# nickgreenquist/cu2rec

Measured on AMD Instinct MI355X. Metric: ratings/sec (SGD updates/sec), higher is better.
Workload: dtype f32

## Files before the change

### cu2rec_amd/csrc/blocksolve.hpp

```cpp
#pragma once

#include <functional>
#include <vector>

#include <hip/hip_runtime.h>

#include <cstddef>
#include <cstdint>

#include "hip_check.hpp"
#include "kernels.hpp"

namespace cu2rec {

constexpr int kBsLinks = 64;
constexpr int kBsTableStride = 2 * kBsLinks + 1;
constexpr int kBsTableFloats = 4 * kBsTableStride;
constexpr int kBsFactorFloats = 3 * 32 * 32;
constexpr int kBsRecFloats = kBsFactorFloats + kBsLinks;
constexpr int kBsCrossFloats = kBsLinks * kBsLinks;
constexpr int kBsMaxSlots = 63;

struct BsBlockDesc {
    int pos0;
    int n_valid;
    int chain;
    int m;
};

struct BsChainDesc {
    int begin, len;
    int blk0;
    int item;
};

struct BsIteration {
    const uint32_t *keys;
    const uint64_t *vals;
    int n_active;
    int n_hot;
    uint32_t item_mask;
    const BsChainDesc *chains;
    const BsBlockDesc *blocks;
    const int *walk_begin;
    const int *item_of_rank;
    const float *tables;
    float log2a, log2c;
    float *Mbuf;
    float *ebuf;
    float *qstart;
    int max_blocks;
    int launch_blocks;
    int la_ranks;
    int la_cap;
    int la_grid;
    float *Nbuf;
    unsigned *status;
    unsigned long long *solve_started;
    const unsigned long long *side_seq;
    unsigned long long side_target;
    unsigned long long *gram_done;
    unsigned long long wait_ticks;
};

float blocksolve_min_rate(float rate);
int blocksolve_lookahead_blocks(int blocks);
int blocksolve_hot_items(const std::vector<double> &rate, int n_active, int rank_limit);

class BlockSolve {
public:
    BlockSolve(int n_hot, const std::vector<double> &rate, double hot_rate, int n_active, int item_bits, int max_batch,
               const int *item_of_rank);
    ~BlockSolve();
    BlockSolve(const BlockSolve &) = delete;
    BlockSolve &operator=(const BlockSolve &) = delete;
    void plan(int slot, const uint32_t *sk, int nb, size_t stride, hipStream_t sched);
    void begin(const SgdArgs &a, hipStream_t stream);
    using SideChains = std::function<void(hipStream_t side, hipEvent_t stop)>;
    void iteration(const SgdArgs &a, int slot, int b, const uint32_t *keys, const uint64_t *vals, bool last, hipStream_t stream,
                   const SideChains &side);
    void join(hipStream_t stream);
    void end(hipStream_t stream);

    const int n_hot;

private:
    int n_active, item_bits, max_batch;
    const int *item_of_rank;
    int max_blocks;
    int launch_blocks;
    int la_ranks = 0;
    int la_cap = 0;
    DeviceBuffer<int> chain_begin[2], walk_begin[2];
    DeviceBuffer<BsChainDesc> chains[2];
    DeviceBuffer<BsBlockDesc> blocks[2];
    DeviceBuffer<float> tables, Mbuf, ebuf, qstart, Nbuf;
    int qstart_ld = 0;
    SgdHyper tables_for{};
    bool tables_valid = false;
    DeviceBuffer<unsigned long long> solve_started, gram_done, side_seq;
    unsigned long long gram_done_target = 0, started_total = 0, side_seq_host = 0;
    hipStream_t upd = nullptr;
    hipEvent_t ev_call = nullptr, ev_upd = nullptr, ev_gram = nullptr;
    BsIteration it{};
    bool device_join = false;
    bool upd_pending = false;
    unsigned *host_status = nullptr;
};

}
```

### cu2rec_amd/csrc/blocksolve_device.hpp

```cpp
#pragma once

#include <hip/hip_runtime.h>

#include "blocksolve.hpp"
#include "sgd_device.hpp"

namespace cu2rec {
namespace bs_dev {

using namespace dev;

constexpr int kB = kBsLinks;
constexpr int kTabAdel = 0, kTabCdel = kBsTableStride, kTabApow = 2 * kBsTableStride, kTabCpow = 3 * kBsTableStride;
constexpr int kH = 32;
constexpr int kMS = 36;

typedef float f32x4 __attribute__((ext_vector_type(4)));
typedef float f32x2 __attribute__((ext_vector_type(2)));
__device__ __forceinline__ f32x4 lds4(const float4 *p) { return *reinterpret_cast<const f32x4 *>(p); }
__device__ __forceinline__ f32x2 lo2(f32x4 v) { return __builtin_shufflevector(v, v, 0, 1); }
__device__ __forceinline__ f32x2 hi2(f32x4 v) { return __builtin_shufflevector(v, v, 2, 3); }
__device__ __forceinline__ f32x2 fma2(f32x2 a, f32x2 b, f32x2 c) { return __builtin_elementwise_fma(a, b, c); }
__device__ __forceinline__ f32x2 dup2(float v) { return f32x2{v, v}; }
typedef unsigned int u32x2 __attribute__((ext_vector_type(2)));

__device__ __forceinline__ unsigned ld_agent(const unsigned *p) {
    return __hip_atomic_load(p, __ATOMIC_RELAXED, __HIP_MEMORY_SCOPE_AGENT);
}
__device__ __forceinline__ unsigned long long ld_agent(const unsigned long long *p) {
    return __hip_atomic_load(p, __ATOMIC_RELAXED, __HIP_MEMORY_SCOPE_AGENT);
}

__device__ __forceinline__ float row_pair_sum(float v) {
    const u32x2 r = __builtin_amdgcn_permlane16_swap(__float_as_uint(v), __float_as_uint(v), false, false);
    return __uint_as_float(r.x) + __uint_as_float(r.y);
}

__device__ __forceinline__ float half_sum(float v) {
    const u32x2 r = __builtin_amdgcn_permlane32_swap(__float_as_uint(v), __float_as_uint(v), false, false);
    return __uint_as_float(r.x) + __uint_as_float(r.y);
}

__device__ __forceinline__ float lane_value(float v, int lane) {
    return __int_as_float(__builtin_amdgcn_readlane(__float_as_int(v), lane));
}

__device__ __forceinline__ float4 zero4() { return make_float4(0.f, 0.f, 0.f, 0.f); }

__device__ __forceinline__ bool chain_is_lookahead(const BsIteration &it, int chain, const BsChainDesc &cd) {
    const int nblk = (cd.len + kB - 1) / kB;
    return chain < it.la_ranks && nblk >= 2 && cd.blk0 + nblk <= it.la_cap;
}

}
}
```

### cu2rec_amd/csrc/blocksolve_gram.hpp

```cpp
#pragma once

#include "blocksolve_device.hpp"
#include "mfma_f32.hpp"

namespace cu2rec {
namespace bs_dev {

constexpr int kGramTabFloats = 2 * kB;
__host__ __device__ inline size_t gram_tile_float4s(int nslots) { return static_cast<size_t>(kB) * (nslots | 1); }

__host__ __device__ inline int gram_tab_offset(int RS) { return max(4 * kB * RS, 5 * kH * kMS); }
__host__ __device__ inline size_t gram_lds_bytes(int nslots, bool with_cross_blocks) {
    const size_t own = static_cast<size_t>(gram_tab_offset(nslots | 1) + kGramTabFloats + kB) * sizeof(float);
    const size_t cross = with_cross_blocks ? 2 * gram_tile_float4s(nslots) * sizeof(float4) : 0;
    return own > cross ? own : cross;
}

__device__ __forceinline__ void gram_block(const SgdArgs &a, const BsIteration &it, int g, float4 *bs_smem) {
    const int wave = threadIdx.x >> 6, lane = threadIdx.x & 63;
    const BsBlockDesc bd = it.blocks[g];
    if (bd.n_valid == 0) return;
    const int nslots = a.nslots, RS = nslots | 1;
    float4 *tile = bs_smem;
    float *Ms = reinterpret_cast<float *>(bs_smem);
    float *Ns = Ms + 2 * kH * kMS;
    float *tab = Ms + gram_tab_offset(RS);
    float *basev = tab + kGramTabFloats;
    const bool mine = lane < bd.n_valid;
    const uint64_t val = it.vals[bd.pos0 + min(lane, bd.n_valid - 1)];
    const int x = static_cast<int>(val >> 32);
    if (wave == 3) {
        const float r0 = (__uint_as_float(static_cast<uint32_t>(val)) - a.global_bias) - a.user_bias[x];
        basev[lane] = mine ? r0 : 0.f;
        tab[lane] = it.tables[kTabApow + lane];
        tab[kB + lane] = it.tables[kTabCpow + lane];
    }
    const int rsub = lane >> 3, cs = lane & 7;
    const int nch = (nslots + 7) >> 3;
    for (int c0 = 0; c0 < nch; c0 += 4) {
        float4 v[2][4];
#pragma unroll
        for (int pp = 0; pp < 2; ++pp) {
            const int xr = __shfl(x, 16 * wave + 8 * pp + rsub);
            const float4 *src = reinterpret_cast<const float4 *>(a.P + static_cast<size_t>(xr) * a.ldp);
#pragma unroll
            for (int c = 0; c < 4; ++c) v[pp][c] = src[min(8 * (c0 + c) + cs, nslots - 1)];
        }
#pragma unroll
        for (int pp = 0; pp < 2; ++pp) {
            const int row = 16 * wave + 8 * pp + rsub;
#pragma unroll
            for (int c = 0; c < 4; ++c) {
                const int slot = 8 * (c0 + c) + cs;
                if (slot < nslots) tile[row * RS + slot] = row < bd.n_valid ? v[pp][c] : zero4();
            }
        }
    }
    __syncthreads();
    const int k = lane & 31, h = lane >> 5;
    f32x16 acc;
#pragma unroll
    for (int i = 0; i < 16; ++i) acc[i] = 0.f;
    if (wave < 3) {
        const int S0 = (nslots + 1) >> 1;
        const float4 *ra = tile + (wave == 1 ? kH + k : k) * RS, *rb = tile + (wave == 0 ? k : kH + k) * RS;
        for (int c = 0; c < S0; c += 2) {
            float4 va[2], vb[2];
#pragma unroll
            for (int i = 0; i < 2; ++i) {
                const int slot = h * S0 + c + i;
                const bool ok = c + i < S0 && slot < nslots;
                const float4 t0 = ra[min(slot, nslots - 1)], t1 = rb[min(slot, nslots - 1)];
                va[i] = ok ? t0 : zero4();
                vb[i] = ok ? t1 : zero4();
            }
#pragma unroll
            for (int i = 0; i < 2; ++i) {
                const float pa[4] = {va[i].x, va[i].y, va[i].z, va[i].w}, pb[4] = {vb[i].x, vb[i].y, vb[i].z, vb[i].w};
#pragma unroll
                for (int e = 0; e < 4; ++e) acc = __builtin_amdgcn_mfma_f32_32x32x2f32(pa[e], pb[e], acc, 0, 0, 0);
            }
        }
    }
    __syncthreads();
    if (wave < 3) {
        const float lr = a.h.lr;
        const int K = (wave == 0 ? 0 : kH) + k;
        const int J0 = (wave == 1 ? kH : 0) + 4 * h;
        const bool row_ok = K < bd.n_valid;
        float *dst = Ns + (wave * kH + k) * kMS + 4 * h;
#pragma unroll
        for (int m = 0; m < 4; ++m) {
            f32x4 out;
#pragma unroll
            for (int e = 0; e < 4; ++e) {
                const int d = K - 1 - (J0 + 8 * m + e);
                const float fd = static_cast<float>(d);
                const float v = lr * (__builtin_amdgcn_exp2f(fd * it.log2c) + __builtin_amdgcn_exp2f(fd * it.log2a) * acc[4 * m + e]);
                out[e] = d >= 0 && row_ok ? v : 0.f;
            }
            *reinterpret_cast<f32x4 *>(dst + 8 * m) = out;
        }
    }
    __syncthreads();
    if (wave == 0) {
    float m[kH];
    {
        const float *Nh = Ns + h * kH * kMS;
        float4 cur[8], nxt[8];
        m[0] = k == 0 ? 1.f : 0.f;
        cur[0] = *reinterpret_cast<const float4 *>(Nh + kMS);
#pragma unroll
        for (int kk = 1; kk < kH; ++kk) {
            if (kk + 1 < kH) {
#pragma unroll
                for (int i4 = 0; i4 < (kk + 4) / 4; ++i4) nxt[i4] = *reinterpret_cast<const float4 *>(Nh + (kk + 1) * kMS + 4 * i4);
            }
            __builtin_amdgcn_sched_barrier(0);
            float s[4] = {kk == k ? 1.f : 0.f, 0.f, 0.f, 0.f};
#pragma unroll
            for (int i4 = 0; i4 < (kk + 3) / 4; ++i4) {
                const float nv[4] = {cur[i4].x, cur[i4].y, cur[i4].z, cur[i4].w};
#pragma unroll
                for (int e = 0; e < 4; ++e)
                    if (4 * i4 + e < kk) s[e] = __builtin_fmaf(-nv[e], m[4 * i4 + e], s[e]);
            }
            m[kk] = (s[0] + s[1]) + (s[2] + s[3]);
            __builtin_amdgcn_sched_barrier(0);
            if (kk + 1 < kH) {
#pragma unroll
                for (int i4 = 0; i4 < (kk + 4) / 4; ++i4) cur[i4] = nxt[i4];
            }
        }
    }
#pragma unroll
    for (int kk = 0; kk < kH; ++kk) Ms[(h * kH + kk) * kMS + k] = m[kk];
    __builtin_amdgcn_wave_barrier();
    f32x16 tacc, macc;
#pragma unroll
    for (int i = 0; i < 16; ++i) tacc[i] = macc[i] = 0.f;
    {
        const float4 *arow = reinterpret_cast<const float4 *>(Ns + (2 * kH + k) * kMS + 16 * h);
#pragma unroll
        for (int t4 = 0; t4 < 4; ++t4) {
            const float4 a4 = arow[t4];
            const float av[4] = {a4.x, a4.y, a4.z, a4.w};
#pragma unroll
            for (int e = 0; e < 4; ++e)
                tacc = __builtin_amdgcn_mfma_f32_32x32x2f32(av[e], Ms[(16 * h + 4 * t4 + e) * kMS + k], tacc, 0, 0, 0);
        }
        const float *mrow = Ms + (kH + k) * kMS + 4 * h;
#pragma unroll
        for (int t4 = 0; t4 < 4; ++t4) {
            const float4 a4 = *reinterpret_cast<const float4 *>(mrow + 8 * t4);
            const float av[4] = {a4.x, a4.y, a4.z, a4.w};
#pragma unroll
            for (int e = 0; e < 4; ++e) macc = __builtin_amdgcn_mfma_f32_32x32x2f32(av[e], tacc[4 * t4 + e], macc, 0, 0, 0);
        }
    }
#pragma unroll
    for (int reg = 0; reg < 16; ++reg) Ns[acc_row(reg, h) * kMS + k] = -macc[reg];
    }
    __syncthreads();
    float *rec = it.Mbuf + static_cast<size_t>(g) * kBsRecFloats;
    {
        const int t = threadIdx.x, row = t >> 3, c4 = t & 7;
        const float *src[3] = {Ms, Ns, Ms + kH * kMS};
#pragma unroll
        for (int q = 0; q < 3; ++q) *reinterpret_cast<f32x4 *>(rec + q * kH * kH + 4 * t) = *reinterpret_cast<const f32x4 *>(src[q] + row * kMS + 4 * c4);
        if (t < kB / 4) *reinterpret_cast<f32x4 *>(rec + kBsFactorFloats + 4 * t) = *reinterpret_cast<const f32x4 *>(basev + 4 * t);
    }
}

__device__ __forceinline__ void gram_cross_block(const SgdArgs &a, const BsIteration &it, int g, float4 *smem) {
    const BsBlockDesc bd = it.blocks[g];
    if (bd.n_valid == 0 || bd.m == 0 || !chain_is_lookahead(it, bd.chain, it.chains[bd.chain])) return;
    const int wave = threadIdx.x >> 6, lane = threadIdx.x & 63, k = lane & 31, h = lane >> 5;
    const int rt = wave >> 1, ct = wave & 1;
    const int nslots = a.nslots, RS = nslots | 1, S0 = (nslots + 1) >> 1;
    float4 *tile_c = smem, *tile_p = smem + kB * RS;
    {
        const int xc = static_cast<int>(it.vals[bd.pos0 + min(lane, bd.n_valid - 1)] >> 32);
        const int xp = static_cast<int>(it.vals[bd.pos0 - kB + lane] >> 32);
        const int rsub = lane >> 3, cs = lane & 7;
        const int nch = (nslots + 7) >> 3;
        for (int c0 = 0; c0 < nch; c0 += 2) {
            float4 vc[2][2], vp[2][2];
#pragma unroll
            for (int pp = 0; pp < 2; ++pp) {
                const int src_lane = 16 * wave + 8 * pp + rsub;
                const float4 *sc = reinterpret_cast<const float4 *>(a.P + static_cast<size_t>(__shfl(xc, src_lane)) * a.ldp);
                const float4 *sp = reinterpret_cast<const float4 *>(a.P + static_cast<size_t>(__shfl(xp, src_lane)) * a.ldp);
#pragma unroll
                for (int c = 0; c < 2; ++c) {
                    vc[pp][c] = sc[min(8 * (c0 + c) + cs, nslots - 1)];
                    vp[pp][c] = sp[min(8 * (c0 + c) + cs, nslots - 1)];
                }
            }
#pragma unroll
            for (int pp = 0; pp < 2; ++pp) {
                const int row = 16 * wave + 8 * pp + rsub;
#pragma unroll
                for (int c = 0; c < 2; ++c) {
                    const int slot = 8 * (c0 + c) + cs;
                    if (slot < nslots) {
                        tile_c[row * RS + slot] = row < bd.n_valid ? vc[pp][c] : zero4();
                        tile_p[row * RS + slot] = vp[pp][c];
                    }
                }
            }
        }
    }
    __syncthreads();
    f32x16 acc;
#pragma unroll
    for (int i = 0; i < 16; ++i) acc[i] = 0.f;
    {
        const float4 *ra = tile_c + (kH * rt + k) * RS, *rb = tile_p + (kH * ct + k) * RS;
        for (int c = 0; c < S0; c += 2) {
            float4 va[2], vb[2];
#pragma unroll
            for (int i = 0; i < 2; ++i) {
                const int slot = h * S0 + c + i;
                const bool ok = c + i < S0 && slot < nslots;
                const float4 t0 = ra[min(slot, nslots - 1)], t1 = rb[min(slot, nslots - 1)];
                va[i] = ok ? t0 : zero4();
                vb[i] = ok ? t1 : zero4();
            }
#pragma unroll
            for (int i = 0; i < 2; ++i) {
                const float pa[4] = {va[i].x, va[i].y, va[i].z, va[i].w}, pb[4] = {vb[i].x, vb[i].y, vb[i].z, vb[i].w};
#pragma unroll
                for (int e = 0; e < 4; ++e) acc = __builtin_amdgcn_mfma_f32_32x32x2f32(pa[e], pb[e], acc, 0, 0, 0);
            }
        }
    }
    const float lr = a.h.lr;
    float *dst = it.Nbuf + static_cast<size_t>(g) * kBsCrossFloats;
    const int j = kH * ct + k;
#pragma unroll
    for (int reg = 0; reg < 16; ++reg) {
        const int i = kH * rt + acc_row(reg, h);
        const float fd = static_cast<float>(kB - 1 + i - j);
        const float v = lr * (__builtin_amdgcn_exp2f(fd * it.log2c) + __builtin_amdgcn_exp2f(fd * it.log2a) * acc[reg]);
        dst[i * kB + j] = i < bd.n_valid ? v : 0.f;
    }
    __syncthreads();
}

}
}
```

### cu2rec_amd/csrc/blocksolve_lookahead.hpp

```cpp
#pragma once

#include "blocksolve_device.hpp"

namespace cu2rec {
namespace bs_dev {

constexpr int kLaPRing = 3, kLaRRing = 2, kLaDepth = 2;
constexpr int kLaNS4 = 17;
constexpr int kLaRec4 = 3 * kH * kMS / 4 + kB * kLaNS4;
constexpr int kLaQ4 = 32;
constexpr int kLaMaxSlots = 29;
__host__ __device__ inline bool la_supported(int nslots) { return nslots >= 1 && nslots <= kLaMaxSlots; }
__host__ __device__ inline size_t la_lds_bytes(int nslots) {
    return (static_cast<size_t>(kLaPRing) * kB * (nslots | 1) + kLaRRing * kLaRec4 + 2 * kLaQ4 + 7 * kB / 4 + (kBsTableFloats + 3) / 4 + 4 + 64) * 16;
}

enum { kSyC0 = 0, kSyC1 = 1, kSyE = 2, kSyG = 3, kSyLdP = 4, kSyLdR = 8, kSyR = 12, kSyAbort = 13 };

template <class Reached>
__device__ __forceinline__ void la_wait_until(unsigned *sy, const BsIteration &it, Reached reached) {
    unsigned polls = 0;
    unsigned long long t0 = 0;
    while (!reached()) {
        __builtin_amdgcn_s_sleep(1);
        if ((++polls & 1023u) == 0) {
            if (t0 == 0) t0 = wall_clock64();
            if (__hip_atomic_load(sy + kSyAbort, __ATOMIC_RELAXED, __HIP_MEMORY_SCOPE_WORKGROUP) != 0u || wall_clock64() - t0 > it.wait_ticks) {
                __hip_atomic_store(sy + kSyAbort, 2u, __ATOMIC_RELAXED, __HIP_MEMORY_SCOPE_WORKGROUP);
                if ((threadIdx.x & 63) == 0) __hip_atomic_store(it.status, 2u, __ATOMIC_RELAXED, __HIP_MEMORY_SCOPE_AGENT);
                break;
            }
        }
    }
    asm volatile("" ::: "memory");
}
__device__ __forceinline__ void la_wait(unsigned *sy, int word, unsigned target, const BsIteration &it) {
    la_wait_until(sy, it, [=] __device__ { return __hip_atomic_load(sy + word, __ATOMIC_RELAXED, __HIP_MEMORY_SCOPE_WORKGROUP) >= target; });
}
__device__ __forceinline__ void la_wait4(unsigned *sy, int word, unsigned target, const BsIteration &it) {
    la_wait_until(sy, it, [=] __device__ {
        typedef unsigned u32x4 __attribute__((ext_vector_type(4)));
        const u32x4 v = __builtin_nontemporal_load((const __attribute__((address_space(3))) u32x4 *)(sy + word));
        asm volatile("" ::: "memory");
        return min(min(v.x, v.y), min(v.z, v.w)) >= target;
    });
}
__device__ __forceinline__ void la_wait2(unsigned *sy, int word, unsigned target, const BsIteration &it) {
    la_wait_until(sy, it, [=] __device__ {
        const u32x2 v = __builtin_nontemporal_load((const __attribute__((address_space(3))) u32x2 *)(sy + word));
        asm volatile("" ::: "memory");
        return min(v.x, v.y) >= target;
    });
}
__device__ __forceinline__ void la_post(unsigned *sy, int word, unsigned value) {
    asm volatile("" ::: "memory");
    if ((threadIdx.x & 63) == 0) __hip_atomic_store(sy + word, value, __ATOMIC_RELAXED, __HIP_MEMORY_SCOPE_WORKGROUP);
}

template <int NSM>
__device__ __forceinline__ void chain_lookahead(const SgdArgs &a, const BsIteration &it, float4 *smem, const BsChainDesc &cd) {
    const int tid = threadIdx.x, wave = tid >> 6, lane = tid & 63;
    const int nslots = a.nslots, RS = nslots | 1;
    const int begin = cd.begin, len = cd.len, nblk = (len + kB - 1) / kB, g0 = cd.blk0, y = cd.item;
    float4 *pring = smem;
    float4 *rring = pring + kLaPRing * kB * RS;
    float4 *qbuf = rring + kLaRRing * kLaRec4;
    float *wbuf = reinterpret_cast<float *>(qbuf + 2 * kLaQ4);
    float *ebl = wbuf + 2 * kB;
    float *tbuf = ebl + 2 * kB;
    float *gbuf = tbuf + kB;
    float *tab = gbuf + 2 * kB;
    unsigned *sy = reinterpret_cast<unsigned *>(tab + ((kBsTableFloats + 3) & ~3));
    f32x4 *sink = reinterpret_cast<f32x4 *>(sy + 16);
    const float lr = a.h.lr;

    if (wave >= 4) {
        const int w = wave - 4;
        __builtin_amdgcn_s_setprio(2);
        constexpr int NQ = (NSM + 3) / 4;
        const int idx0 = w * kB * NQ + lane;
        const int row0 = idx0 / nslots, slot0 = idx0 - row0 * nslots;
        const int drow = kB / nslots, dslot = kB - drow * nslots;
        auto load_val = [&](int i) -> uint64_t { return it.vals[begin + min(kB * i + lane, len - 1)]; };
        struct LaStage {
            f32x4 v[NQ], r[8];
            uint64_t next_val;
        };
        auto issue = [&](LaStage &st, int i, uint64_t val) {
            const int ic = min(i, nblk - 1);
            st.next_val = load_val(min(i + kLaDepth, nblk - 1));
            const int x = static_cast<int>(val >> 32);
            int row = row0, slot = slot0;
#pragma unroll
            for (int j = 0; j < NQ; ++j) {
                const int xr = __shfl(x, min(row, kB - 1));
                st.v[j] = reinterpret_cast<const f32x4 *>(a.P + static_cast<size_t>(xr) * a.ldp)[slot];
                slot += dslot, row += drow;
                if (slot >= nslots) slot -= nslots, ++row;
            }
            const f32x4 *src = w < 2 ? reinterpret_cast<const f32x4 *>(it.Mbuf + static_cast<size_t>(g0 + ic) * kBsRecFloats) + 384 * w
                                     : reinterpret_cast<const f32x4 *>(it.Nbuf + static_cast<size_t>(g0 + max(ic, 1)) * kBsCrossFloats) + 512 * (w - 2);
#pragma unroll
            for (int j = 0; j < 8; ++j) {
                const int at = w < 2 && j >= 6 ? 768 - 384 * w + (lane & 15) : lane + 64 * j;
                st.r[j] = src[at];
            }
        };
        auto commit = [&](const LaStage &st, int i) {
            if (i >= kLaPRing) {
                la_wait2(sy, kSyC0, static_cast<unsigned>(i - kLaPRing + 1), it);
            }
            {
                f32x4 *tile = reinterpret_cast<f32x4 *>(pring + (i % kLaPRing) * kB * RS);
                int row = row0, slot = slot0;
                const f32x4 z = {0.f, 0.f, 0.f, 0.f};
#pragma unroll
                for (int j = 0; j < NQ; ++j) {
                    f32x4 *dst = row < kB ? tile + row * RS + slot : sink + lane;
                    *dst = kB * i + row < len ? st.v[j] : z;
                    slot += dslot, row += drow;
                    if (slot >= nslots) slot -= nslots, ++row;
                }
            }
            la_post(sy, kSyLdP + w, static_cast<unsigned>(i + 1));
            if (i >= kLaRRing) la_wait(sy, kSyR, static_cast<unsigned>(i - kLaRRing + 1), it);
            f32x4 *rr = reinterpret_cast<f32x4 *>(rring + (i % kLaRRing) * kLaRec4);
            if (w < 2) {
#pragma unroll
                for (int j = 0; j < 6; ++j) {
                    const int idx = 384 * w + lane + 64 * j;
                    rr[((idx >> 8) * kH + ((idx >> 3) & 31)) * (kMS / 4) + (idx & 7)] = st.r[j];
                }
                if (w == 0 && lane < 16) {
                    float *col = reinterpret_cast<float *>(rr) + (4 * lane) * kMS + kH;
#pragma unroll
                    for (int e = 0; e < 4; ++e) col[e * kMS] = st.r[6][e];
                }
            } else {
                f32x4 *nl = rr + 3 * kH * kMS / 4;
#pragma unroll
                for (int j = 0; j < 8; ++j) {
                    const int idx = 512 * (w - 2) + lane + 64 * j;
                    nl[(idx >> 4) * kLaNS4 + (idx & 15)] = st.r[j];
                }
            }
            la_post(sy, kSyLdR + w, static_cast<unsigned>(i + 1));
        };
        static_assert(kLaDepth == 2, "two stages: four wavefronts x two blocks x 15 KB in flight");
        LaStage st[kLaDepth];
        {
            uint64_t v0[kLaDepth];
#pragma unroll
            for (int t = 0; t < kLaDepth; ++t) v0[t] = load_val(min(t, nblk - 1));
#pragma unroll
            for (int t = 0; t < kLaDepth; ++t) issue(st[t], t, v0[t]);
        }
        __syncthreads();
        for (int m0 = 0; m0 < nblk; m0 += kLaDepth) {
#pragma unroll
            for (int u = 0; u < kLaDepth; ++u) {
                const int i = m0 + u;
                if (i < nblk) commit(st[u], i);
                issue(st[u], i + kLaDepth, st[u].next_val);
            }
        }
        return;
    }

    if (wave == 3) {
        __syncthreads();
        __builtin_amdgcn_s_setprio(2);
        for (int i = 0; i < nblk; ++i) {
            const int src = max(i - 1, 0);
            la_wait4(sy, kSyLdP, static_cast<unsigned>(i + 1), it);
            if (src > 0) la_wait2(sy, kSyC0, static_cast<unsigned>(src), it);
            const float4 *prow = pring + (i % kLaPRing) * kB * RS + lane * RS;
            const float4 *qv = qbuf + (src & 1) * kLaQ4;
            constexpr int NH2 = (NSM + 1) / 2;
            f32x2 acc[4] = {dup2(0.f), dup2(0.f), dup2(0.f), dup2(0.f)};
#pragma unroll
            for (int hh = 0; hh < 2; ++hh) {
                f32x4 pv[NH2], qq[NH2];
#pragma unroll
                for (int j = 0; j < NH2; ++j) {
                    pv[j] = lds4(prow + min(hh * NH2 + j, nslots - 1));
                    qq[j] = lds4(qv + min(hh * NH2 + j, kLaQ4 - 1));
                }
                __builtin_amdgcn_sched_barrier(0);
#pragma unroll
                for (int j = 0; j < NH2; ++j) {
                    if (hh * NH2 + j < NSM) {
                        acc[2 * (j & 1)] = fma2(lo2(pv[j]), lo2(qq[j]), acc[2 * (j & 1)]);
                        acc[2 * (j & 1) + 1] = fma2(hi2(pv[j]), hi2(qq[j]), acc[2 * (j & 1) + 1]);
                    }
                }
                __builtin_amdgcn_sched_barrier(0);
            }
            acc[0] += acc[2];
            acc[1] += acc[3];
            const f32x2 ds = acc[0] + acc[1];
            gbuf[(i & 1) * kB + lane] = ds.x + ds.y;
            la_post(sy, kSyG, static_cast<unsigned>(i + 1));
        }
        return;
    }

    if (wave >= 1) {
        const int c = wave - 1;
        constexpr int NP = (NSM + 7) / 8, NPW = (NP + 1) / 2;
        const int sl = lane & 7, kg = lane >> 3;
        f32x4 q4[NPW];
        const f32x4 *qsrc = reinterpret_cast<const f32x4 *>(a.Q + static_cast<size_t>(y) * a.ldq);
#pragma unroll
        for (int pp = 0; pp < NPW; ++pp) {
            const int slot = 8 * (2 * pp + c) + sl;
            const f32x4 v = qsrc[min(slot, nslots - 1)];
            q4[pp] = slot < nslots ? v : f32x4{0.f, 0.f, 0.f, 0.f};
            if (kg < 2 && slot < kLaQ4) *reinterpret_cast<f32x4 *>(qbuf + kg * kLaQ4 + slot) = kg == 0 ? q4[pp] : f32x4{0.f, 0.f, 0.f, 0.f};
        }
        __syncthreads();
        __builtin_amdgcn_s_setprio(2);
        for (int i = 0; i < nblk; ++i) {
            const int n = min(kB, len - kB * i);
            const float adel_n = tab[kTabAdel + n];
            la_wait(sy, kSyE, static_cast<unsigned>(i + 1), it);
            const float4 *tile = pring + (i % kLaPRing) * kB * RS;
            const float4 *wv = reinterpret_cast<const float4 *>(wbuf + (i & 1) * kB) + 2 * kg;
            float *qdst = it.qstart + static_cast<size_t>(g0 + i) * a.ldq;
            const f32x4 wb0 = lds4(wv), wb1 = lds4(wv + 1);
            f32x4 tb[NPW][8];
#pragma unroll
            for (int pp = 0; pp < NPW; ++pp) {
                const float4 *colp = tile + (8 * kg) * RS + min(8 * (2 * pp + c) + sl, nslots - 1);
#pragma unroll
                for (int r = 0; r < 8; ++r) tb[pp][r] = lds4(colp + r * RS);
            }
            __builtin_amdgcn_sched_barrier(0);
#pragma unroll
            for (int pp = 0; pp < NPW; ++pp) {
                const int slot = 8 * (2 * pp + c) + sl;
                const bool ok = slot < nslots;
                if (ok && kg == 0) *reinterpret_cast<f32x4 *>(qdst + 4 * slot) = q4[pp];
                f32x2 ulo = dup2(0.f), uhi = dup2(0.f);
#pragma unroll
                for (int r = 0; r < 8; ++r) {
                    const f32x2 ww = dup2(r < 4 ? wb0[r & 3] : wb1[r & 3]);
                    ulo = fma2(ww, lo2(tb[pp][r]), ulo);
                    uhi = fma2(ww, hi2(tb[pp][r]), uhi);
                }
                float u[4] = {ulo.x, ulo.y, uhi.x, uhi.y};
#pragma unroll
                for (int e = 0; e < 4; ++e) {
                    u[e] += __int_as_float(__builtin_amdgcn_update_dpp(0, __float_as_int(u[e]), 0x128, 0xf, 0xf, false));
                    u[e] = half_sum(row_pair_sum(u[e]));
                }
                const f32x4 qo = q4[pp];
                q4[pp] = ok ? f32x4{(qo.x - adel_n * qo.x) + u[0], (qo.y - adel_n * qo.y) + u[1], (qo.z - adel_n * qo.z) + u[2],
                                    (qo.w - adel_n * qo.w) + u[3]}
                            : f32x4{0.f, 0.f, 0.f, 0.f};
                if (ok && kg == 0) *reinterpret_cast<f32x4 *>(qbuf + ((i + 1) & 1) * kLaQ4 + slot) = q4[pp];
            }
            la_post(sy, kSyC0 + c, static_cast<unsigned>(i + 1));
        }
        if (kg == 0) {
            f32x4 *qd = reinterpret_cast<f32x4 *>(a.Q + static_cast<size_t>(y) * a.ldq);
#pragma unroll
            for (int pp = 0; pp < NPW; ++pp) {
                const int slot = 8 * (2 * pp + c) + sl;
                if (slot < nslots) qd[slot] = q4[pp];
            }
        }
        return;
    }

    const int k = lane;
    for (int i = k; i < kBsTableFloats; i += 64) tab[i] = it.tables[i];
    if (k < 16) sy[k] = 0u;
    float b_cur = a.item_bias[y], b_prev = b_cur;
    asm volatile("" ::"v"(b_cur));
    __syncthreads();
    __builtin_amdgcn_s_setprio(3);
    const int kr = k & 31;
    const bool upper = k >= kH;
    f32x4 m4[16], n4[16];
    float base;
    auto take_record = [&](int i) {
        la_wait4(sy, kSyLdR, static_cast<unsigned>(i + 1), it);
        const float4 *rr = rring + (i % kLaRRing) * kLaRec4;
        const float *Mt = reinterpret_cast<const float *>(rr);
        const float4 *mlo = reinterpret_cast<const float4 *>(Mt + ((upper ? kH : 0) + kr) * kMS);
        const float4 *mhi = reinterpret_cast<const float4 *>(Mt + (2 * kH + kr) * kMS);
        const float4 *nrow = rr + 3 * kH * kMS / 4 + k * kLaNS4;
#pragma unroll
        for (int j = 0; j < 8; ++j) {
            m4[j] = lds4(mlo + j);
            const f32x4 hi = lds4(mhi + j);
            m4[8 + j] = upper ? hi : f32x4{0.f, 0.f, 0.f, 0.f};
        }
#pragma unroll
        for (int j = 0; j < 16; ++j) n4[j] = lds4(nrow + j);
        base = Mt[k * kMS + kH];
        la_post(sy, kSyR, static_cast<unsigned>(i + 1));
    };
    take_record(0);
    for (int i = 0; i < nblk; ++i) {
        const int n = min(kB, len - kB * i);
        f32x2 tacc[2] = {dup2(0.f), dup2(0.f)};
        if (i > 0) {
            const float4 *ev = reinterpret_cast<const float4 *>(ebl + ((i - 1) & 1) * kB);
            f32x4 e4[16];
#pragma unroll
            for (int j = 0; j < 16; ++j) e4[j] = lds4(ev + j);
            __builtin_amdgcn_sched_barrier(0);
#pragma unroll
            for (int j = 0; j < 16; ++j) {
                tacc[0] = fma2(lo2(n4[j]), lo2(e4[j]), tacc[0]);
                tacc[1] = fma2(hi2(n4[j]), hi2(e4[j]), tacc[1]);
            }
        }
        const f32x2 ts = tacc[0] + tacc[1];
        const float t0 = ts.x + ts.y;
        const int kd = i > 0 ? k + kB : k;
        const float adel_k = tab[kTabAdel + kd], cdel_k = tab[kTabCdel + kd];
        const float bsrc = i > 0 ? b_prev : b_cur;
        la_wait(sy, kSyG, static_cast<unsigned>(i + 1), it);
        const float gd = gbuf[(i & 1) * kB + k];
        const float pre = k < n ? (base - (bsrc - cdel_k * bsrc)) - (gd - adel_k * gd) : 0.f;
        tbuf[k] = pre - t0;
        asm volatile("" ::: "memory");
        __builtin_amdgcn_wave_barrier();
        f32x2 eacc[2] = {dup2(0.f), dup2(0.f)};
        {
            const float4 *tv = reinterpret_cast<const float4 *>(tbuf);
            f32x4 t4[16];
#pragma unroll
            for (int j = 0; j < 16; ++j) t4[j] = lds4(tv + j);
            __builtin_amdgcn_sched_barrier(0);
#pragma unroll
            for (int j = 0; j < 16; ++j) {
                eacc[0] = fma2(lo2(m4[j]), lo2(t4[j]), eacc[0]);
                eacc[1] = fma2(hi2(m4[j]), hi2(t4[j]), eacc[1]);
            }
        }
        const f32x2 es = eacc[0] + eacc[1];
        const float e = k < n ? es.x + es.y : 0.f;
        const int back = max(n - 1 - k, 0);
        ebl[(i & 1) * kB + k] = e;
        wbuf[(i & 1) * kB + k] = k < n ? lr * tab[kTabApow + back] * e : 0.f;
        la_post(sy, kSyE, static_cast<unsigned>(i + 1));
        it.ebuf[static_cast<size_t>(g0 + i) * kB + k] = e;
        if (i + 1 < nblk) take_record(i + 1);
        const float bs = row_sum16(k < n ? lr * tab[kTabCpow + back] * e : 0.f);
        const float cdel_n = tab[kTabCdel + n];
        const float b_next = (b_cur - cdel_n * b_cur) + ((lane_value(bs, 0) + lane_value(bs, 16)) + (lane_value(bs, 32) + lane_value(bs, 48)));
        b_prev = b_cur;
        b_cur = b_next;
    }
    if (k == 0) a.item_bias[y] = b_cur;
}

}
}
```

### cu2rec_amd/csrc/blocksolve_solve.hpp

```cpp
#pragma once

#include "blocksolve_device.hpp"

namespace cu2rec {
namespace bs_dev {

constexpr int kSolTabStride = kB + 1, kSolTabFloats = 4 * kSolTabStride;
constexpr int kSolTabAdel = 0, kSolTabCdel = kSolTabStride, kSolTabApow = 2 * kSolTabStride, kSolTabCpow = 3 * kSolTabStride;
constexpr int kRing = 2;
constexpr int kDepth = 4;

template <int N>
struct Stage {
    f32x4 rows[N];
    f32x4 m4[3];
    float base;
    uint64_t next_val;
};

__host__ __device__ inline int solve_slot_f4(int nslots) { return kB * (nslots | 1) + 3 * kH * kMS / 4; }

__host__ __device__ inline size_t solve_lds_bytes(int nslots, int sw) {
    return (static_cast<size_t>(kRing) * solve_slot_f4(nslots) + 4 * sw + 8 + 2 * kB + 8 * kB / 4 + (kSolTabFloats + 3) / 4 + 8 + 1) * 16;
}

__device__ __forceinline__ void solvers_meet(unsigned *meet, unsigned target, int lane) {
    __builtin_amdgcn_fence(__ATOMIC_RELEASE, "workgroup");
    if (lane == 0) __hip_atomic_fetch_add(meet, 1u, __ATOMIC_RELAXED, __HIP_MEMORY_SCOPE_WORKGROUP);
    while (__hip_atomic_load(meet, __ATOMIC_RELAXED, __HIP_MEMORY_SCOPE_WORKGROUP) < target) __builtin_amdgcn_s_sleep(1);
    __builtin_amdgcn_fence(__ATOMIC_ACQUIRE, "workgroup");
}

template <int SW>
__device__ __forceinline__ void solve_chain(const SgdArgs &a, const BsIteration &it, float4 *bs_smem, const BsChainDesc &cd) {
    const int begin = cd.begin, len = cd.len;
    if (len <= 0) return;
    const int nblk = (len + kB - 1) / kB;
    const int g0 = cd.blk0;
    const int nslots = a.nslots, RS = nslots | 1;
    const int S4 = solve_slot_f4(nslots);
    const bool long_chain = nblk > kDepth;
    const int n_intervals = long_chain ? (nblk + kDepth - 1) / kDepth * kDepth : kDepth;
    float4 *smem = bs_smem;
    const int tid = threadIdx.x;

    if (tid >= 256) {
        __builtin_amdgcn_s_setprio(2);
        constexpr int NLT = SW;
        const int lt = tid - 256, tr = lt >> 2, tp = lt & 3;
        auto load_val = [&](int t) -> uint64_t { return it.vals[begin + min(kB * t + tr, len - 1)]; };
        auto issue_rows = [&](Stage<NLT> &s, int t, uint64_t val) {
            s.next_val = load_val(t + kDepth);
            const f32x4 *row = reinterpret_cast<const f32x4 *>(a.P + static_cast<size_t>(static_cast<uint32_t>(val >> 32)) * a.ldp);
#pragma unroll
            for (int i = 0; i < NLT; ++i) s.rows[i] = row[min(tp + 4 * i, nslots - 1)];
        };
        auto issue_rec = [&](Stage<NLT> &s, int t) {
            const float *rec = it.Mbuf + static_cast<size_t>(g0 + min(t, nblk - 1)) * kBsRecFloats;
            const f32x4 *mg = reinterpret_cast<const f32x4 *>(rec);
#pragma unroll
            for (int q = 0; q < 3; ++q) s.m4[q] = mg[q * 256 + lt];
            s.base = rec[kBsFactorFloats + (lt & 63)];
        };
        auto issue = [&](Stage<NLT> &s, int t, uint64_t val) {
            issue_rows(s, t, val);
            issue_rec(s, t);
        };
        auto commit = [&](const Stage<NLT> &s, int t) {
            f32x4 *sl = reinterpret_cast<f32x4 *>(smem + (t % kRing) * S4);
            const bool rv = kB * t + tr < len;
            const f32x4 z = {0.f, 0.f, 0.f, 0.f};
#pragma unroll
            for (int i = 0; i < NLT; ++i) {
                const int slot = tp + 4 * i;
                if (slot < nslots) sl[tr * RS + slot] = rv ? s.rows[i] : z;
            }
            f32x4 *mt = sl + kB * RS;
#pragma unroll
            for (int q = 0; q < 3; ++q) {
                const int item = q * 256 + lt;
                mt[(item >> 3) * (kMS / 4) + (item & 7)] = s.m4[q];
            }
            if (lt < kB) reinterpret_cast<float *>(mt)[lt * kMS + kH] = kB * t + lt < len ? s.base : 0.f;
        };
        Stage<NLT> st[kDepth];
        if (long_chain) {
            uint64_t v[kDepth];
#pragma unroll
            for (int t = 0; t < kDepth; ++t) v[t] = load_val(t);
#pragma unroll
            for (int t = 0; t < kDepth; ++t) issue(st[t], t, v[t]);
            commit(st[0], 0);
            issue(st[0], kDepth, st[0].next_val);
            __syncthreads();
            for (int m0 = 0; m0 < n_intervals; m0 += kDepth) {
#pragma unroll
                for (int u = 0; u < kDepth; ++u) {
                    const int m = m0 + u;
                    Stage<NLT> &s = st[(u + 1) % kDepth];
                    commit(s, m + 1);
                    issue(s, m + 1 + kDepth, s.next_val);
                    __syncthreads();
                }
            }
        } else {
            uint64_t v[kDepth];
#pragma unroll
            for (int t = 0; t < kDepth; ++t) v[t] = load_val(min(t, nblk - 1));
#pragma unroll
            for (int t = 0; t < kDepth; ++t)
                if (t < nblk) issue(st[t], t, v[t]);
            commit(st[0], 0);
            __syncthreads();
#pragma unroll
            for (int u = 0; u < kDepth; ++u) {
                if (u + 1 < kDepth && u + 1 < nblk) commit(st[(u + 1) % kDepth], u + 1);
                __syncthreads();
            }
        }
        return;
    }

    __builtin_amdgcn_s_setprio(3);
    const int w = tid >> 6, k = tid & 63;
    constexpr int NP = (SW + 7) / 8;
    float4 *qrow = smem + kRing * S4;
    float4 *dpart = qrow + 4 * SW + 8;
    float4 *epart = dpart + kB;
    float *rbuf = reinterpret_cast<float *>(epart + kB) + w * kB;
    float *wbuf = reinterpret_cast<float *>(epart + kB) + (4 + w) * kB;
    float *tab = reinterpret_cast<float *>(epart + kB) + 8 * kB;
    float4 *zrow = reinterpret_cast<float4 *>(tab) + (kSolTabFloats + 3) / 4;
    unsigned *meet = reinterpret_cast<unsigned *>(zrow + 8);
    if (w == 0) {
        for (int i = k; i < kSolTabFloats; i += 64) tab[i] = it.tables[(i / kSolTabStride) * kBsTableStride + i % kSolTabStride];
        if (k < 8) zrow[k] = zero4();
        if (k == 0) *meet = 0u;
    }
    unsigned met = 0;
    const int y = cd.item;
    const int sl = k & 7, kg = k >> 3;
    f32x4 q4[NP];
    const f32x4 *qsrc = reinterpret_cast<const f32x4 *>(a.Q + static_cast<size_t>(y) * a.ldq);
#pragma unroll
    for (int p = 0; p < NP; ++p) {
        const int sq = 8 * p + sl, slot = w * SW + sq;
        const f32x4 v = qsrc[min(slot, nslots - 1)];
        q4[p] = sq < SW && slot < nslots ? v : f32x4{0.f, 0.f, 0.f, 0.f};
        if (kg == 0 && sq < SW) *reinterpret_cast<f32x4 *>(qrow + slot) = q4[p];
    }
    float b = a.item_bias[y];
    const float lr = a.h.lr;
    const int kr = k & 31;
    const bool upper = k >= kH;
    __syncthreads();
    for (int m = 0; m < n_intervals; ++m) {
        const bool live = m < nblk;
        const int n = min(kB, len - kB * m);
        const float4 *tile = smem + (m % kRing) * S4;
        const float *Mt = reinterpret_cast<const float *>(tile + kB * RS);
        float base = 0.f, adel_k = 0.f, cdel_k = 0.f, apr = 0.f, cpr = 0.f, adel_n = 0.f, cdel_n = 0.f;
        f32x4 mq[4];
        if (live) {
            const float4 *mrow = w < 2 ? reinterpret_cast<const float4 *>(Mt + ((upper ? kH : 0) + kr) * kMS + 16 * w)
                                       : (upper ? reinterpret_cast<const float4 *>(Mt + (2 * kH + kr) * kMS + 16 * (w - 2)) : zrow);
#pragma unroll
            for (int t = 0; t < 4; ++t) mq[t] = lds4(mrow + t);
            base = Mt[k * kMS + kH];
            const int back = max(n - 1 - k, 0);
            adel_k = tab[kSolTabAdel + k], cdel_k = tab[kSolTabCdel + k];
            apr = tab[kSolTabApow + back], cpr = tab[kSolTabCpow + back];
            adel_n = tab[kSolTabAdel + n], cdel_n = tab[kSolTabCdel + n];
            const float4 *prow = tile + k * RS;
            f32x4 pv[SW], qv[SW];
#pragma unroll
            for (int i = 0; i < SW; ++i) {
                pv[i] = lds4(prow + min(w * SW + i, nslots - 1));
                qv[i] = lds4(qrow + w * SW + i);
            }
            f32x2 dacc[2] = {dup2(0.f), dup2(0.f)};
#pragma unroll
            for (int i = 0; i < SW; ++i) {
                dacc[0] = fma2(lo2(pv[i]), lo2(qv[i]), dacc[0]);
                dacc[1] = fma2(hi2(pv[i]), hi2(qv[i]), dacc[1]);
            }
            const f32x2 ds = dacc[0] + dacc[1];
            reinterpret_cast<float *>(dpart)[4 * k + w] = ds.x + ds.y;
        }
        met += 4;
        solvers_meet(meet, met, k);
        if (live) {
            const f32x4 d4 = lds4(dpart + k);
            const float d = (d4.x + d4.y) + (d4.z + d4.w);
            const float rhs = k < n ? (base - (b - cdel_k * b)) - (d - adel_k * d) : 0.f;
            rbuf[k] = rhs;
            __builtin_amdgcn_wave_barrier();
            const float4 *rv = reinterpret_cast<const float4 *>(rbuf) + 4 * w;
            f32x2 eacc[2] = {dup2(0.f), dup2(0.f)};
#pragma unroll
            for (int t = 0; t < 4; ++t) {
                const f32x4 r4 = lds4(rv + t);
                eacc[0] = fma2(lo2(mq[t]), lo2(r4), eacc[0]);
                eacc[1] = fma2(hi2(mq[t]), hi2(r4), eacc[1]);
            }
            const f32x2 es = eacc[0] + eacc[1];
            reinterpret_cast<float *>(epart)[4 * k + w] = es.x + es.y;
        }
        met += 4;
        solvers_meet(meet, met, k);
        if (live) {
            const f32x4 e4 = lds4(epart + k);
            const float e = (e4.x + e4.y) + (e4.z + e4.w);
            if (w == 0) {
                const float e0 = k < n ? e : 0.f;
                const f32x4 e4v = {e0, dpp_move<0x55>(e0), dpp_move<0xAA>(e0), dpp_move<0xFF>(e0)};
                if ((k & 3) == 0) {
                    float *dst = it.ebuf + static_cast<size_t>(g0 + m) * kB + k;
                    *reinterpret_cast<f32x4 *>(dst) = e4v;
                }
            }
            wbuf[k] = k < n ? lr * apr * e : 0.f;
            const float bs = row_sum16(k < n ? lr * cpr * e : 0.f);
            b = (b - cdel_n * b) + ((lane_value(bs, 0) + lane_value(bs, 16)) + (lane_value(bs, 32) + lane_value(bs, 48)));
            __builtin_amdgcn_wave_barrier();
            float *qdst = it.qstart + static_cast<size_t>(g0 + m) * a.ldq;
            const float4 *wv = reinterpret_cast<const float4 *>(wbuf) + 2 * kg;
#pragma unroll
            for (int p = 0; p < NP; ++p) {
                const int sq = 8 * p + sl, slot = w * SW + sq;
                const bool ok = sq < SW && slot < nslots;
                if (ok && kg == 0) *reinterpret_cast<f32x4 *>(qdst + 4 * slot) = q4[p];
                const float4 *colp = tile + (8 * kg) * RS + min(slot, nslots - 1);
                f32x4 tb[8], wb[2];
#pragma unroll
                for (int i = 0; i < 8; ++i) tb[i] = lds4(colp + i * RS);
                wb[0] = lds4(wv), wb[1] = lds4(wv + 1);
                f32x2 ulo = dup2(0.f), uhi = dup2(0.f);
#pragma unroll
                for (int i = 0; i < 8; ++i) {
                    const f32x2 ww = dup2(wb[i >> 2][i & 3]);
                    ulo = fma2(ww, lo2(tb[i]), ulo);
                    uhi = fma2(ww, hi2(tb[i]), uhi);
                }
                float u[4] = {ulo.x, ulo.y, uhi.x, uhi.y};
#pragma unroll
                for (int c = 0; c < 4; ++c) {
                    u[c] += __int_as_float(__builtin_amdgcn_update_dpp(0, __float_as_int(u[c]), 0x128, 0xf, 0xf, false));
                    u[c] = half_sum(row_pair_sum(u[c]));
                }
                const f32x4 qo = q4[p];
                q4[p] = ok ? f32x4{(qo.x - adel_n * qo.x) + u[0], (qo.y - adel_n * qo.y) + u[1], (qo.z - adel_n * qo.z) + u[2],
                                   (qo.w - adel_n * qo.w) + u[3]}
                           : f32x4{0.f, 0.f, 0.f, 0.f};
                if (kg == 0 && sq < SW) *reinterpret_cast<f32x4 *>(qrow + slot) = q4[p];
            }
        }
        __syncthreads();
    }
    {
        if (kg == 0) {
            f32x4 *qdst = reinterpret_cast<f32x4 *>(a.Q + static_cast<size_t>(y) * a.ldq);
#pragma unroll
            for (int p = 0; p < NP; ++p) {
                const int sq = 8 * p + sl, slot = w * SW + sq;
                if (sq < SW && slot < nslots) qdst[slot] = q4[p];
            }
        }
        if (tid == 0) a.item_bias[y] = b;
    }
}

}
}
```

Before: 1.771 billion.

## Pack lower-triangular factor tiles in block records to shrink global traffic

The per-block record written by the gram kernel now stores the two 32x32 triangular factor tiles packed into 288 float4 instead of two full tiles, alongside the M21 tile and base errors. The solve and lookahead loaders are remapped to unpack the packed triangles into their LDS layout, zeroing the upper triangles once per slot up front. This cuts the record bytes each chain step reads from global memory, at the cost of more complex index mapping and precomputed scatter destinations held in registers.

```diff
diff --git a/cu2rec_amd/csrc/blocksolve.hpp b/cu2rec_amd/csrc/blocksolve.hpp
--- a/cu2rec_amd/csrc/blocksolve.hpp
+++ b/cu2rec_amd/csrc/blocksolve.hpp
@@ -16,8 +16,8 @@
 constexpr int kBsLinks = 64;
 constexpr int kBsTableStride = 2 * kBsLinks + 1;
 constexpr int kBsTableFloats = 4 * kBsTableStride;
-constexpr int kBsFactorFloats = 3 * 32 * 32;
-constexpr int kBsRecFloats = kBsFactorFloats + kBsLinks;
+constexpr int kBsFactorFloats = 4 * (256 + 288);
+constexpr int kBsRecFloats = kBsFactorFloats + kBsLinks + 64;
 constexpr int kBsCrossFloats = kBsLinks * kBsLinks;
 constexpr int kBsMaxSlots = 63;
 
diff --git a/cu2rec_amd/csrc/blocksolve_device.hpp b/cu2rec_amd/csrc/blocksolve_device.hpp
--- a/cu2rec_amd/csrc/blocksolve_device.hpp
+++ b/cu2rec_amd/csrc/blocksolve_device.hpp
@@ -47,6 +47,32 @@
 
 __device__ __forceinline__ float4 zero4() { return make_float4(0.f, 0.f, 0.f, 0.f); }
 
+constexpr int kRecM21 = 0, kRecTri = 4 * 256, kRecBase = kBsFactorFloats;
+constexpr int kRecTri4 = 288;
+static_assert(kRecTri + 4 * kRecTri4 == kBsFactorFloats && kRecBase + kB + 64 == kBsRecFloats && kBsRecFloats == 4 * 576, "the record: M21 | triangles | base errors | unused");
+
+struct TriPlace {
+    int tile, row, c4;
+};
+__device__ __forceinline__ TriPlace tri_place(int t) {
+    const int R = t >> 3, c = t & 7, g = R >> 2;
+    if (R >= kH) return TriPlace{1, R - 4, c};
+    if (R >= 28 || c <= g) return TriPlace{0, R, c};
+    return TriPlace{1, 27 - R, c - g - 1};
+}
+__device__ __forceinline__ int tri_place_lds(int t) {
+    const TriPlace p = tri_place(t);
+    return (2 * p.tile * kH + p.row) * (kMS / 4) + p.c4;
+}
+__device__ __forceinline__ void tri_zero_upper(f32x4 *tiles, int slot4, int t) {
+    const int k = (t >> 3) & (kH - 1), c4 = t & 7;
+    if (t < 256 && c4 > (k >> 2)) {
+        const f32x4 z = {0.f, 0.f, 0.f, 0.f};
+#pragma unroll
+        for (int q = 0; q < 4; ++q) tiles[(q >> 1) * slot4 + (2 * (q & 1) * kH + k) * (kMS / 4) + c4] = z;
+    }
+}
+
 __device__ __forceinline__ bool chain_is_lookahead(const BsIteration &it, int chain, const BsChainDesc &cd) {
     const int nblk = (cd.len + kB - 1) / kB;
     return chain < it.la_ranks && nblk >= 2 && cd.blk0 + nblk <= it.la_cap;
diff --git a/cu2rec_amd/csrc/blocksolve_gram.hpp b/cu2rec_amd/csrc/blocksolve_gram.hpp
--- a/cu2rec_amd/csrc/blocksolve_gram.hpp
+++ b/cu2rec_amd/csrc/blocksolve_gram.hpp
@@ -165,10 +165,14 @@
     float *rec = it.Mbuf + static_cast<size_t>(g) * kBsRecFloats;
     {
         const int t = threadIdx.x, row = t >> 3, c4 = t & 7;
-        const float *src[3] = {Ms, Ns, Ms + kH * kMS};
-#pragma unroll
-        for (int q = 0; q < 3; ++q) *reinterpret_cast<f32x4 *>(rec + q * kH * kH + 4 * t) = *reinterpret_cast<const f32x4 *>(src[q] + row * kMS + 4 * c4);
-        if (t < kB / 4) *reinterpret_cast<f32x4 *>(rec + kBsFactorFloats + 4 * t) = *reinterpret_cast<const f32x4 *>(basev + 4 * t);
+        *reinterpret_cast<f32x4 *>(rec + kRecM21 + 4 * t) = *reinterpret_cast<const f32x4 *>(Ns + row * kMS + 4 * c4);
+        const TriPlace p0 = tri_place(t);
+        *reinterpret_cast<f32x4 *>(rec + kRecTri + 4 * t) = *reinterpret_cast<const f32x4 *>(Ms + (p0.tile * kH + p0.row) * kMS + 4 * p0.c4);
+        if (t < kRecTri4 - 256) {
+            const TriPlace p1 = tri_place(256 + t);
+            *reinterpret_cast<f32x4 *>(rec + kRecTri + 4 * (256 + t)) = *reinterpret_cast<const f32x4 *>(Ms + (p1.tile * kH + p1.row) * kMS + 4 * p1.c4);
+        }
+        if (t < kB / 4) *reinterpret_cast<f32x4 *>(rec + kRecBase + 4 * t) = *reinterpret_cast<const f32x4 *>(basev + 4 * t);
     }
 }
 
diff --git a/cu2rec_amd/csrc/blocksolve_lookahead.hpp b/cu2rec_amd/csrc/blocksolve_lookahead.hpp
--- a/cu2rec_amd/csrc/blocksolve_lookahead.hpp
+++ b/cu2rec_amd/csrc/blocksolve_lookahead.hpp
@@ -10,6 +10,9 @@
 constexpr int kLaRec4 = 3 * kH * kMS / 4 + kB * kLaNS4;
 constexpr int kLaQ4 = 32;
 constexpr int kLaMaxSlots = 29;
+constexpr int kLaRec4Mem = kBsRecFloats / 4;
+constexpr int kLaRecLoads = (kLaRec4Mem + kBsCrossFloats / 4 + 255) / 256;
+static_assert(kLaRec4Mem % 64 == 0 && kLaRecLoads == 7, "record and cross block: 1,600 float4 over four wavefronts, the seam between them on a wavefront's load");
 __host__ __device__ inline bool la_supported(int nslots) { return nslots >= 1 && nslots <= kLaMaxSlots; }
 __host__ __device__ inline size_t la_lds_bytes(int nslots) {
     return (static_cast<size_t>(kLaPRing) * kB * (nslots | 1) + kLaRRing * kLaRec4 + 2 * kLaQ4 + 7 * kB / 4 + (kBsTableFloats + 3) / 4 + 4 + 64) * 16;
@@ -82,8 +85,23 @@
         const int row0 = idx0 / nslots, slot0 = idx0 - row0 * nslots;
         const int drow = kB / nslots, dslot = kB - drow * nslots;
         auto load_val = [&](int i) -> uint64_t { return it.vals[begin + min(kB * i + lane, len - 1)]; };
+        int rdst[kLaRRing][kLaRecLoads];
+        f32x4 *lds4w = reinterpret_cast<f32x4 *>(smem);
+#pragma unroll
+        for (int j = 0; j < kLaRecLoads; ++j) {
+            const int v = 256 * j + 64 * w + lane;
+            const int ci = v - kLaRec4Mem;
+            const int off = v < 256 ? (kH + (v >> 3)) * (kMS / 4) + (v & 7)
+                          : v < 256 + kRecTri4 ? tri_place_lds(v - 256)
+                          : 3 * kH * kMS / 4 + (ci >> 4) * kLaNS4 + (ci & 15);
+            const bool keep = v < 256 + kRecTri4 || (ci >= 0 && ci < kBsCrossFloats / 4);
+#pragma unroll
+            for (int r = 0; r < kLaRRing; ++r)
+                rdst[r][j] = keep ? static_cast<int>(rring - smem) + r * kLaRec4 + off : static_cast<int>(sink - lds4w) + lane;
+        }
+        tri_zero_upper(reinterpret_cast<f32x4 *>(rring), kLaRec4, tid - 256);
         struct LaStage {
-            f32x4 v[NQ], r[8];
+            f32x4 v[NQ], r[kLaRecLoads];
             uint64_t next_val;
         };
         auto issue = [&](LaStage &st, int i, uint64_t val) {
@@ -98,15 +116,15 @@
                 slot += dslot, row += drow;
                 if (slot >= nslots) slot -= nslots, ++row;
             }
-            const f32x4 *src = w < 2 ? reinterpret_cast<const f32x4 *>(it.Mbuf + static_cast<size_t>(g0 + ic) * kBsRecFloats) + 384 * w
-                                     : reinterpret_cast<const f32x4 *>(it.Nbuf + static_cast<size_t>(g0 + max(ic, 1)) * kBsCrossFloats) + 512 * (w - 2);
-#pragma unroll
-            for (int j = 0; j < 8; ++j) {
-                const int at = w < 2 && j >= 6 ? 768 - 384 * w + (lane & 15) : lane + 64 * j;
-                st.r[j] = src[at];
+            const f32x4 *rec = reinterpret_cast<const f32x4 *>(it.Mbuf + static_cast<size_t>(g0 + ic) * kBsRecFloats);
+            const f32x4 *cross = reinterpret_cast<const f32x4 *>(it.Nbuf + static_cast<size_t>(g0 + max(ic, 1)) * kBsCrossFloats);
+#pragma unroll
+            for (int j = 0; j < kLaRecLoads; ++j) {
+                const int v0 = 256 * j + 64 * w;
+                st.r[j] = v0 < kLaRec4Mem ? rec[v0 + lane] : cross[min(v0 - kLaRec4Mem + lane, kBsCrossFloats / 4 - 1)];
             }
         };
-        auto commit = [&](const LaStage &st, int i) {
+        auto commit = [&](const LaStage &st, int i, int slot) {
             if (i >= kLaPRing) {
                 la_wait2(sy, kSyC0, static_cast<unsigned>(i - kLaPRing + 1), it);
             }
@@ -124,29 +142,16 @@
             }
             la_post(sy, kSyLdP + w, static_cast<unsigned>(i + 1));
             if (i >= kLaRRing) la_wait(sy, kSyR, static_cast<unsigned>(i - kLaRRing + 1), it);
-            f32x4 *rr = reinterpret_cast<f32x4 *>(rring + (i % kLaRRing) * kLaRec4);
-            if (w < 2) {
-#pragma unroll
-                for (int j = 0; j < 6; ++j) {
-                    const int idx = 384 * w + lane + 64 * j;
-                    rr[((idx >> 8) * kH + ((idx >> 3) & 31)) * (kMS / 4) + (idx & 7)] = st.r[j];
-                }
-                if (w == 0 && lane < 16) {
-                    float *col = reinterpret_cast<float *>(rr) + (4 * lane) * kMS + kH;
-#pragma unroll
-                    for (int e = 0; e < 4; ++e) col[e * kMS] = st.r[6][e];
-                }
-            } else {
-                f32x4 *nl = rr + 3 * kH * kMS / 4;
-#pragma unroll
-                for (int j = 0; j < 8; ++j) {
-                    const int idx = 512 * (w - 2) + lane + 64 * j;
-                    nl[(idx >> 4) * kLaNS4 + (idx & 15)] = st.r[j];
-                }
+#pragma unroll
+            for (int j = 0; j < kLaRecLoads; ++j) lds4w[rdst[slot][j]] = st.r[j];
+            if (w == 0 && lane >= 32 && lane < 48) {
+                float *col = reinterpret_cast<float *>(rring + slot * kLaRec4) + 4 * (lane - 32) * kMS + kH;
+#pragma unroll
+                for (int e = 0; e < 4; ++e) col[e * kMS] = st.r[2][e];
             }
             la_post(sy, kSyLdR + w, static_cast<unsigned>(i + 1));
         };
-        static_assert(kLaDepth == 2, "two stages: four wavefronts x two blocks x 15 KB in flight");
+        static_assert(kLaDepth == 2 && kLaDepth % kLaRRing == 0, "two stages: four wavefronts x two blocks x 14 KB in flight; stage u fills record slot u");
         LaStage st[kLaDepth];
         {
             uint64_t v0[kLaDepth];
@@ -160,7 +165,7 @@
 #pragma unroll
             for (int u = 0; u < kLaDepth; ++u) {
                 const int i = m0 + u;
-                if (i < nblk) commit(st[u], i);
+                if (i < nblk) commit(st[u], i, u % kLaRRing);
                 issue(st[u], i + kLaDepth, st[u].next_val);
             }
         }
diff --git a/cu2rec_amd/csrc/blocksolve_solve.hpp b/cu2rec_amd/csrc/blocksolve_solve.hpp
--- a/cu2rec_amd/csrc/blocksolve_solve.hpp
+++ b/cu2rec_amd/csrc/blocksolve_solve.hpp
@@ -48,6 +48,9 @@
         __builtin_amdgcn_s_setprio(2);
         constexpr int NLT = SW;
         const int lt = tid - 256, tr = lt >> 2, tp = lt & 3;
+        const int tri2 = lt < kRecTri4 - 256 ? 256 + lt : lt;
+        const int tri_dst1 = tri_place_lds(lt), tri_dst2 = tri_place_lds(tri2);
+        tri_zero_upper(reinterpret_cast<f32x4 *>(smem + kB * RS), S4, lt);
         auto load_val = [&](int t) -> uint64_t { return it.vals[begin + min(kB * t + tr, len - 1)]; };
         auto issue_rows = [&](Stage<NLT> &s, int t, uint64_t val) {
             s.next_val = load_val(t + kDepth);
@@ -58,9 +61,10 @@
         auto issue_rec = [&](Stage<NLT> &s, int t) {
             const float *rec = it.Mbuf + static_cast<size_t>(g0 + min(t, nblk - 1)) * kBsRecFloats;
             const f32x4 *mg = reinterpret_cast<const f32x4 *>(rec);
-#pragma unroll
-            for (int q = 0; q < 3; ++q) s.m4[q] = mg[q * 256 + lt];
-            s.base = rec[kBsFactorFloats + (lt & 63)];
+            s.m4[0] = mg[kRecM21 / 4 + lt];
+            s.m4[1] = mg[kRecTri / 4 + lt];
+            s.m4[2] = mg[kRecTri / 4 + tri2];
+            s.base = rec[kRecBase + (lt & 63)];
         };
         auto issue = [&](Stage<NLT> &s, int t, uint64_t val) {
             issue_rows(s, t, val);
@@ -76,11 +80,9 @@
                 if (slot < nslots) sl[tr * RS + slot] = rv ? s.rows[i] : z;
             }
             f32x4 *mt = sl + kB * RS;
-#pragma unroll
-            for (int q = 0; q < 3; ++q) {
-                const int item = q * 256 + lt;
-                mt[(item >> 3) * (kMS / 4) + (item & 7)] = s.m4[q];
-            }
+            mt[(kH + (lt >> 3)) * (kMS / 4) + (lt & 7)] = s.m4[0];
+            mt[tri_dst1] = s.m4[1];
+            mt[tri_dst2] = s.m4[2];
             if (lt < kB) reinterpret_cast<float *>(mt)[lt * kMS + kH] = kB * t + lt < len ? s.base : 0.f;
         };
         Stage<NLT> st[kDepth];
```

Result: no change. 1.781 billion, median of 6 (+0.5%).
